# hidasib/GRU4Rec

Hardware: AMD Instinct MI355X
Metric: mini-batches/sec (gru4rec.py:661), RSC15-shaped batch=128 n_sample=2048 BPR-max (higher is better)
Workload: dtype f32

## Files before the change

gru4rec_amd/csrc/g4r_host_create.hpp:

```cpp

int g4r_device_count(void) {
    int n = 0;
    if (hipGetDeviceCount(&n) != hipSuccess) return 0;
    return n;
}
const char* g4r_last_error(void) { return g_err.c_str(); }
#ifndef G4R_HIPCC_VERSION
#define G4R_HIPCC_VERSION "unknown"
#endif
const char* g4r_version(void) { return "gru4rec_hip 0.4 (gfx950; hipcc " G4R_HIPCC_VERSION "; isa-audited)"; }
int g4r_sizeof_config(void) { return (int)sizeof(g4r_config); }

static int build_lean_args(g4r_model* m) {
    DevModel& d = m->dm;
    const StepKernels& k = m->kern;
    const int L = d.n_layers;
    std::vector<LeanV> av(L); std::vector<LeanH> ah(L); std::vector<LeanDa> aa(L); std::vector<LeanDy> ay(L);
    const bool constrained = d.embed_mode == G4R_EMBED_CONSTRAINED;
    bool any_layer = false;
    for (int l = 0; l < L; ++l) {
        if (k.fwd[l] != FWD_LEAN) continue;
        any_layer = true;
        LeanV& v = av[l]; memset(&v, 0, sizeof(v));
        v.Wx = d.dense_p + d.offWx[l]; v.Wrz = d.dense_p + d.offWrz[l]; v.Bh = d.dense_p + d.offBh[l];
// ... 42 lines not shown
        m->h_leanB = q;
        if (dalloc(m, &m->d_leanB, (size_t)1)) return -1;
        HIPCHK(hipMemcpyAsync(m->d_leanB, &m->h_leanB, sizeof(LeanB), hipMemcpyHostToDevice, m->stream));
    }
    if (k.update == UP_LEAN) {
        LeanU u; memset(&u, 0, sizeof(u));
        u.mp = nullptr; u.st = d.st; u.Wy = d.Wy; u.E = d.E; u.accWy = d.accWy; u.accE = d.accE; u.velWy = d.velWy; u.velE = d.velE;
        u.By = d.By; u.accBy = d.accBy; u.velBy = d.velBy; u.dAx = d.dAx; u.dAy = d.dAy; u.dABy = d.dABy;
        u.dense_p = d.dense_p; u.dense_acc = d.dense_acc; u.dense_vel = d.dense_vel; u.yin0 = d.yin0; u.meta = d.cur_in + 2 * d.B;
        u.dbg = d.dbgclk; u.dbgtile = d.dbgtile; u.n_items = d.n_items; u.constrained = constrained ? 1 : 0; u.wE = d.Ein; u.wY = d.Dtop;
        u.lr = d.lr; u.mom = d.mom; u.lmbd = d.lmbd;
        m->h_leanU = u;
        const std::vector<DenseTile> tiles = dense_tiles(d, 16, 64);
        m->ntiles16 = (int)tiles.size();
        const size_t nslot = cdiv((long long)G4R_OWN_SLOTS * d.R * 16 * sizeof(int), (long long)sizeof(DenseTile));
        if (dalloc(m, &m->d_tiles16, tiles.size() + nslot) || dalloc(m, &m->d_leanU, (size_t)1)) return -1;
        d.own_pos = m->sw.owner_scan_in_update ? nullptr : (int*)(m->d_tiles16 + tiles.size());
        m->h_leanU.own_on = d.own_pos ? 1 : 0;
        const bool pays = cdiv(d.R, LOSS_NW) > G4R_OWN_WINDOW_MINWG;
        m->own_window = d.own_pos && d.R <= G4R_OWN_WINDOW_MAXR && (m->sw.owner_window > 0 || (m->sw.owner_window < 0 && pays));
        HIPCHK(hipMemcpyAsync(m->d_tiles16, tiles.data(), tiles.size() * sizeof(DenseTile), hipMemcpyHostToDevice, m->stream));
        HIPCHK(hipStreamSynchronize(m->stream));
    }
    HIPCHK(hipStreamSynchronize(m->stream));
    return 0;
}

static KernelSwitches read_switches(const g4r_config& cfg) {
    KernelSwitches w;
    w.no_lean = getenv("G4R_NO_LEAN") != nullptr; w.no_mt = getenv("G4R_NO_MT") != nullptr; w.no_bmt = getenv("G4R_NO_BMT") != nullptr;
    w.no_merge = getenv("G4R_NO_MERGE") != nullptr; w.owner_scan_in_update = env_int("G4R_OWNER_SCAN", 0) != 0;
    w.owner_window = env_int("G4R_OWNER_WINDOW", -1);
    w.score_b_split = env_int("G4R_SCORE_B_SPLIT", 1) != 0;
    w.allow_lean_update = env_int("G4R_LEAN_UPDATE", 1) != 0; w.defer = env_int("G4R_DEFER", cfg.defer_updates) != 0;
    w.p2_geo = env_int("G4R_P2_GEO", -1); w.ba_geo = env_int("G4R_BA_GEO", -1);
    w.wide2 = env_int("G4R_WIDE2", -1); w.p1_ks = env_int("G4R_P1_KS", 128); w.bb_ks = env_int("G4R_BB_KS", 0);
    const char* skip = getenv("G4R_SKIP_KN");
    w.skip_kn = skip ? strtoull(skip, nullptr, 0) : 0ull;
    w.trace = getenv("G4R_TRACE") != nullptr;
    return w;
}

int g4r_create(const g4r_config* cfg, g4r_model** out) {
    if (!cfg || !out) return fail("null argument");
    if (cfg->n_layers < 1 || cfg->n_layers > G4R_MAX_LAYERS) return fail("n_layers out of range");
    if (cfg->batch_size < 1 || cfg->n_items < 1) return fail("batch_size / n_items must be positive");
    for (int l = 0; l < cfg->n_layers; ++l)
        if (cfg->layers[l] % 4 != 0 || cfg->layers[l] < 4 || cfg->layers[l] > 1024)
            return fail("layer sizes must be multiples of 4 in [4, 1024]");
    if (cfg->embed_mode == G4R_EMBED_SEPARATE && (cfg->embedding % 4 != 0 || cfg->embedding < 4 || cfg->embedding > 1024))
        return fail("embedding must be a multiple of 4 in [4, 1024]");
    if (cfg->embed_mode != G4R_EMBED_CONSTRAINED && cfg->embed_mode != G4R_EMBED_SEPARATE && cfg->embed_mode != G4R_EMBED_ONEHOT)
        return fail("unsupported embedding mode");
    if (cfg->embed_mode == G4R_EMBED_ONEHOT && 3 * cfg->layers[0] > 1024)
        return fail("one-hot input: 3 * layers[0] must be <= 1024 (row width of the Wx[0] table)");
    if (cfg->loss < 0 || cfg->loss > G4R_LOSS_XE_LOGIT) return fail("unsupported loss");
    if (cfg->smoothing != 0.f && cfg->loss != G4R_LOSS_XE && cfg->loss != G4R_LOSS_XE_LOGIT) return fail("smoothing needs a cross-entropy loss");
    if (cfg->hidden_act == G4R_ACT_SOFTMAX_LOGIT) return fail("softmax_logit is not a hidden activation");
    if (cfg->adapt < 0 || cfg->adapt > G4R_ADAPT_NONE) return fail("unknown adapt");
    if (cfg->grad_cap < 0.f) return fail("grad_cap must be >= 0");
    if (cfg->hidden_act == G4R_ACT_SOFTMAX) return fail("softmax is not a hidden activation");
    int ndev = g4r_device_count();
    if (ndev <= 0) return fail("no HIP device visible: the gfx950 path has no CPU fallback");
    if (cfg->device < 0 || cfg->device >= ndev) return fail("device ordinal out of range");
    HIPCHK(hipSetDevice(cfg->device));
    int n_cu = 0;
// ... 213 lines not shown
```

gru4rec_amd/csrc/g4r_host_debug.hpp:

```cpp
int g4r_get_debug(g4r_model* m, const char* name, float* host, int64_t count) {
    if (!m || !name || !host) return fail("null argument");
    HIPCHK(hipSetDevice(m->cfg.device));
    DevModel& d = m->dm;
    const StepKernels& k = m->kern;
    std::string s(name);
    const float* p = nullptr; int64_t n = 0;
    int l = 0;
    if (!s.empty() && isdigit((unsigned char)s.back())) { l = s.back() - '0'; s.pop_back(); }
    if (l >= d.n_layers) return fail("layer out of range");
    const int64_t bd = (int64_t)d.B * d.D[l];
    if (s == "scores") { p = d.Sc; n = (int64_t)d.B * d.ldSc; }
    else if (s == "dSx") { p = d.dSx + (size_t)((m->gstep - 1) & d.defer_mask) * (size_t)d.dSx_stride; n = (int64_t)d.B * d.Ein; }
    else if (s == "dSy") { p = d.dSy + (size_t)((m->gstep - 1) & d.defer_mask) * (size_t)d.dSy_stride; n = (int64_t)d.ldSc * d.Dtop; }
    else if (s == "dSBy") { p = d.dSBy + (size_t)((m->gstep - 1) & d.defer_mask) * (size_t)d.dSBy_stride; n = d.ldSc; }
    else if (s == "defer_stats") {
        if (count < 4) return fail("count");
        double rows = 0, bias = 0;
        if (m->defer_on) {
            std::vector<unsigned> st(2048);
            HIPCHK(hipStreamSynchronize(m->stream));
            HIPCHK(hipMemcpy(st.data(), d.dstat, st.size() * sizeof(unsigned), hipMemcpyDeviceToHost));
            for (size_t i = 0; i < st.size(); i += 2) { rows += st[i]; bias += st[i + 1]; }
        }
        host[0] = (float)rows; host[1] = (float)bias; host[2] = m->defer_on ? 1.f : 0.f; host[3] = (float)(d.defer_mask + 1);
// ... 46 lines not shown
    else if (s == "ldSc") { if (count < 1) return fail("count"); host[0] = (float)d.ldSc; return 0; }
    else if (s == "wide_mask") {
        if (count < 1) return fail("count");
        int mk = k.wide_dense ? 16 : 0;
        for (int l = 0; l < d.n_layers; ++l) mk |= k.wg[l].use;
        host[0] = (float)mk; return 0;
    }
    else if (s == "deep_geo") {
        if (count < 1) return fail("count");
        host[0] = (float)(k.p2_deep[0] + 2 * k.ba_deep[0]); return 0;
    }
    else if (s == "score_mt") { if (count < 1) return fail("count"); host[0] = k.score_fwd == SF_MT ? 272.f : 0.f; return 0; }
    else if (s == "score_bmt") { if (count < 1) return fail("count"); host[0] = (float)k.bmt_slabs; return 0; }
    else if (s == "lean") {
        if (count < 4) return fail("count");
        int mk = 0;
        for (int l = 0; l < d.n_layers; ++l) mk |= k.fwd[l] == FWD_LEAN ? 1 << l : 0;
        host[0] = (float)mk; host[1] = k.score_fwd == SF_LEAN ? 1.f : 0.f; host[2] = k.score_bwd == SB_LEAN ? 1.f : 0.f;
        host[3] = k.update == UP_LEAN ? 1.f : 0.f;
        return 0;
    }
    else if (s == "kernels") {
        const int ML = G4R_MAX_LAYERS;
        const int tail[] = {k.score_fwd, k.loss_spec, k.loss_long, k.loss_quads, k.score_bwd, k.kch, k.ksplit, k.bmt_slabs, k.update, k.chunks, k.wide_dense, k.finish_rows};
        if (count < 4 * ML + 12) return fail("count");
        for (int i = 0; i < 4 * ML + 12; ++i) host[i] = i < 4 * ML ? 0.f : (float)tail[i - 4 * ML];
        for (int l = 0; l < d.n_layers; ++l) {
            host[l] = (float)k.fwd[l]; host[ML + l] = (float)k.bwd[l]; host[2 * ML + l] = (float)(k.p2_deep[l] + 2 * k.ba_deep[l]); host[3 * ML + l] = (float)k.wg[l].use;
        }
        return 0;
    }
    else if (s == "generic") { if (count < 1) return fail("count"); host[0] = (float)d.generic; return 0; }
    else if (s == "score_b_split") { if (count < 1) return fail("count"); host[0] = (float)k.score_a_host; return 0; }
    else if (s == "n_cu") { if (count < 1) return fail("count"); host[0] = (float)m->n_cu; return 0; }
    else if (s == "ksplit") { if (count < 1) return fail("count"); host[0] = (float)d.ksplit; return 0; }
    else if (s == "dev_syncs") { if (count < 1) return fail("count"); host[0] = (float)m->n_dev_syncs; return 0; }
    else if (s == "dense_count") { if (count < 1) return fail("count"); host[0] = (float)d.dense_count; return 0; }
    else if (s == "occ_score_tile") {
        if (count < 1) return fail("count");
        int nb = 0;
        for (size_t lds = SMEM_SF2; lds >= SMEM_SF2 - 2048; lds -= 512) {
            HIPCHK(hipOccupancyMaxActiveBlocksPerMultiprocessor(&nb, (const void*)k_score_fwd_t2, GT_NTH, lds));
            fprintf(stderr, "[g4r] k_score_fwd_t2 dynamic LDS %zu -> %d workgroups per CU\n", lds, nb);
        }
        host[0] = (float)nb;
        return 0;
    }
    else if (s == "graph_mode") {
        if (count < 1) return fail("count");
        host[0] = m->gexec ? 1.f : (m->gexec_head ? 2.f : 0.f);
        return 0;
    }
    else return fail(std::string("unknown debug buffer ") + name);
    if (count != n) return fail(std::string("size mismatch for debug buffer ") + name + " expected " + std::to_string(n));
    HIPCHK(hipStreamSynchronize(m->stream));
    HIPCHK(hipMemcpy(host, p, n * sizeof(float), hipMemcpyDeviceToHost));
    return 0;
}

int g4r_debug_loss_rows(g4r_model* m, float* scores, int64_t count, int32_t M, float* lossrow) {
    if (!m || !scores || !lossrow) return fail("null argument");
    DevModel& d = m->dm;
    if (count != (int64_t)d.B * d.ldSc) return fail("size mismatch for the score rows: expected " + std::to_string((int64_t)d.B * d.ldSc));
    if (M < 1 || M > d.B) return fail("M outside [1, batch_size]");
    HIPCHK(hipSetDevice(m->cfg.device));
    HIPCHK(hipStreamSynchronize(m->stream));
// ... 158 lines not shown
```

gru4rec_amd/csrc/g4r_host_model.hpp:

```cpp
static thread_local std::string g_err;
static int fail(const std::string& s) { g_err = s; return -1; }
void g4r_set_error(const char* fmt, ...) {
    char buf[1024];
    va_list ap;
    va_start(ap, fmt);
    vsnprintf(buf, sizeof(buf), fmt, ap);
    va_end(ap);
    g_err = buf;
}
#define HIPCHK(x)                                                                                        \
    do {                                                                                                 \
        hipError_t e_ = (x);                                                                             \
        if (e_ != hipSuccess)                                                                            \
            return fail(std::string(#x) + ": " + hipGetErrorString(e_) + " @" + std::to_string(__LINE__)); \
    } while (0)
#define NCCLCHK(x)                                                                                         \
    do {                                                                                                   \
        ncclResult_t e_ = (x);                                                                             \
        if (e_ != ncclSuccess)                                                                             \
            return fail(std::string(#x) + ": " + ncclGetErrorString(e_) + " @" + std::to_string(__LINE__)); \
    } while (0)

enum { KN_GRU_P1 = 0, KN_GRU_P2, KN_SCORE_FWD, KN_LOSS, KN_SCORE_BWD, KN_BWD_PRE, KN_BWD_A, KN_BWD_B, KN_DENSE, KN_ALLREDUCE,
       KN_DENSE_APPLY, KN_SPARSE, KN_UPDATE, KN_BWD_FUSED, KN_FWD_FUSED, KN_GATE, KN_FLUSH, KN_SCAN, KN_FINISH, KN_GRU_V, KN_GRU_H, KN_GRU_DA, KN_GRU_DY, KN_OWNER_WINDOW, KN_COUNT };
static const char* KN_NAMES[KN_COUNT] = {"k_gru_p1", "k_gru_p2", "k_score_fwd", "k_loss_rows", "k_score_bwd", "k_gru_bwd_pre",
                                         "k_gru_bwd_a", "k_gru_bwd_b", "k_dense_grad", "rccl_allreduce", "k_dense_apply",
                                         "k_sparse_update", "k_update", "k_gru_bwd", "k_gru_fwd", "k_gru_gate", "k_sparse_flush", "k_defer_scan", "k_finish_rows", "k_gru_v", "k_gru_h", "k_gru_da", "k_gru_dy", "k_owner_window"};

struct EvRec { int kn; hipEvent_t a, b; };

struct KernelSwitches {
    bool no_lean = false;
    bool no_mt = false, no_bmt = false;
    bool no_merge = false;
    bool allow_lean_update = true;
    bool score_b_split = true;
    bool owner_scan_in_update = false;
    int owner_window = -1;
    bool defer = false;
    int p2_geo = -1, ba_geo = -1;
    int wide2 = -1, p1_ks = 128, bb_ks = 0;
    unsigned long long skip_kn = 0;
    bool trace = false;
};
enum GruFwdKind { FWD_LEAN = 0 , FWD_FUSED = 1 , FWD_P1S = 2 ,
                  FWD_P1_N64 = 3, FWD_P1_N32 = 4 };
enum GruBwdKind { BWD_LEAN = 0 , BWD_FUSED = 1 , BWD_ONEHOT = 2, BWD_BW = 3, BWD_B = 4 };
enum ScoreFwdKind { SF_LEAN = 0 , SF_MT = 1 , SF_T3 = 2, SF_T2 = 3, SF_K64 = 4, SF_K128 = 5  };
enum ScoreBwdKind { SB_LEAN = 0 , SB_BMT = 1 , SB_BWD2 = 2 , SB_W = 3, SB_N = 4  };
enum UpdateKind { UP_LEAN = 0 , UP_MERGED = 1 , UP_SPLIT = 2 };
struct WideGeo { int use = 0, ny = 1, nh = 1, kys = 0, khs = 0, bbn = 1, bbk = 0; };
struct StepKernels {
    int fwd[G4R_MAX_LAYERS], bwd[G4R_MAX_LAYERS];
    int p2_deep[G4R_MAX_LAYERS], ba_deep[G4R_MAX_LAYERS];
    WideGeo wg[G4R_MAX_LAYERS];
    int score_fwd;
    int loss_spec, loss_long, loss_quads;
    int score_bwd;
    int score_a_host;
    int kch, ksplit;
    int bmt_slabs;
    int nblkA, nblkB, ndtA, ndtB, nrtB;
    int update;
    int chunks;
    int wide_dense;
    int finish_rows;
};

template <class T>
struct DevBuf {
    T* p = nullptr;
    int64_t cap = 0;
    int reserve(g4r_model* m, int64_t n);
};

struct g4r_model {
    g4r_config cfg;
    DevModel dm;
    DevModel* d_dm = nullptr;
    int n_cu = 256;
    KernelSwitches sw;
    StepKernels kern;
    hipStream_t stream = nullptr;
    std::vector<void*> allocs;
    int *d_in = nullptr, *d_out = nullptr, *d_M = nullptr, *d_cmaps = nullptr;
    unsigned char* d_reset = nullptr;
    float* d_loss = nullptr;
    int64_t T = 0, loss_cap = 0;
    std::vector<int64_t> compact_steps;
    int* d_ST = nullptr;
    float *d_P = nullptr, *d_lqt = nullptr, *d_lqs = nullptr;
    int64_t gl = 0;
// ... 309 lines not shown
    }
    const bool lean_s = !sw.no_lean && Dt <= LN_MAXD && Dt % 4 == 0 && !wide && !dma && B < 65536 && d.ldSc < 65536;
    k.score_fwd = lean_s ? SF_LEAN : mt ? SF_MT : dma ? SF_T3 : (wide && Dt % T2_BK == 0) ? SF_T2 : wide ? SF_K64 : SF_K128;
    k.loss_spec = (d.final_act == G4R_ACT_ELU && d.loss == G4R_LOSS_BPR_MAX) ? 1 : (d.final_act == G4R_ACT_SOFTMAX && d.loss == G4R_LOSS_XE) ? 2
                : (d.final_act == G4R_ACT_ELU && d.loss == G4R_LOSS_TOP1_MAX) ? 3 : 0;
    k.loss_long = (size_t)(2 * d.ldSc + 18 * LOSS_NW) * sizeof(float) > (size_t)(156 * 1024);
    k.loss_quads = d.ldSc >= 4 * LOSS_T;
    const bool bwd2 = wide && Dt % 64 == 0;
    const bool top_tiles = k.bwd[top] != BWD_LEAN && k.bwd[top] != BWD_FUSED;
    if (!sw.no_bmt && bwd2 && top_tiles && Dt % 128 == 0 && Dt <= 512 && d.ldSc % BMT_WA == 0 && d.ldSc <= 0xFFFF && B <= 0xFFFF) {
        const int ntA = d.ldSc / BMT_WA * (Dt / 32), den = cdiv(B, 64) * (Dt / 128), ks = ntA / den;
        if (ntA % den == 0 && ntA % 8 == 0 && ntA <= n_cu && ntA * 8 >= n_cu * 7 && BMT_WA % (Dt / 32) == 0 && 4 * (BMT_WA / (Dt / 32)) <= 256 &&
            ks >= 2 && ks <= 24 && d.ldSc % ks == 0 && (d.ldSc / ks) % 32 == 0 && d.ldSc / ks <= 2048)
            k.bmt_slabs = ks;
    }
    k.score_bwd = (lean_s && B <= 128) ? SB_LEAN : k.bmt_slabs ? SB_BMT : bwd2 ? SB_BWD2 : wide ? SB_W : SB_N;
    k.score_a_host = (sw.score_b_split && k.score_bwd == SB_LEAN && k.bwd[top] == BWD_LEAN) ? 1 : 0;
    const int slabs_target = top_tiles ? 17 : 9;
    k.kch = GT_BK * std::max(1, (cdiv(d.ldSc, GT_BK) + slabs_target / 2) / slabs_target);
    if (k.score_bwd == SB_LEAN) k.kch = 128;
    else if (k.score_bwd == SB_BMT) k.kch = d.ldSc / k.bmt_slabs;
    else if (k.score_bwd == SB_BWD2) {
        const int ndt = Dt / 64, nrt = cdiv(B, 64), nA = cdiv(d.ldSc, 64) * ndt;
        double best = 2.0;
        for (int ks = 12; ks <= 24; ++ks) {
            const int kch = (cdiv(d.ldSc, ks) + 7) & ~7;
            if (cdiv(d.ldSc, kch) != ks) continue;
            const double rounds = (double)(nA + ks * nrt * ndt) / n_cu;
            const double waste = (std::ceil(rounds) - rounds) / std::ceil(rounds) + 1e-3 * std::abs(ks - 17);
            if (waste < best) { best = waste; k.kch = kch; }
        }
    }
    k.ksplit = cdiv(d.ldSc, k.kch);
    const int TB = wide ? 64 : 32;
    k.ndtA = cdiv(Dt + 1, TB); k.nblkA = cdiv(d.ldSc, TB) * k.ndtA;
    k.ndtB = cdiv(Dt, TB); k.nrtB = cdiv(B, TB); k.nblkB = k.ksplit * k.nrtB * k.ndtB;
    const int w = std::max(Dt, d.Ein);
    k.chunks = w <= 256 ? 1 : (w <= 512 ? 2 : 4);
    const bool dy0_parts = (k.wg[0].use & 8) != 0;
    const bool merged = !d.generic && !sw.no_merge && k.chunks <= 2 && !k.wide_dense;
    const bool lean_u = !sw.no_lean && sw.allow_lean_update && merged && d.apply_dense_inplace && B <= 128 && k.chunks == 1 && !defer_on && d.xmode == 0 &&
                        !d.touched && !dy0_parts && d.R < 65536 && cdiv(d.R, 8) < 65536 && dense_tiles(d, 16, 64).size() < 65536;
    k.update = lean_u ? UP_LEAN : merged ? UP_MERGED : UP_SPLIT;
    k.finish_rows = dy0_parts && !k.wide_dense;
    return k;
}
static int sync_dm(g4r_model* m) {
    HIPCHK(hipMemcpyAsync(m->d_dm, &m->dm, sizeof(DevModel), hipMemcpyHostToDevice, m->stream));
    HIPCHK(hipStreamSynchronize(m->stream));
    return 0;
}
```

gru4rec_amd/csrc/g4r_host_step.hpp:

```cpp
extern "C++" {
struct StepLauncher {
    g4r_model* m;
    hipStream_t s;
    std::vector<EvRec>* recs;
    size_t evi = 0;
    int kn = -1;
    hipEvent_t ev_a = nullptr, ev_b = nullptr;
    StepLauncher(g4r_model* m_, std::vector<EvRec>* recs_) : m(m_), s(m_->stream), recs(recs_) {}
    void use(int kn_, hipEvent_t a, hipEvent_t b) { kn = kn_; ev_a = a; ev_b = b; }
    void open(int kn_) {
        if (m->sw.trace) { fprintf(stderr, "[g4r] launch %s\n", KN_NAMES[kn_]); fflush(stderr); }
        use(kn_, nullptr, nullptr);
        if (!recs) return;
        while (m->evs.size() < evi + 2) { hipEvent_t e; (void)hipEventCreate(&e); m->evs.push_back(e); }
        use(kn_, m->evs[evi], m->evs[evi + 1]);
        evi += 2;
        recs->push_back(EvRec{kn_, ev_a, ev_b});
    }
    bool skipped() const { return m->sw.skip_kn && kn >= 0 && ((m->sw.skip_kn >> kn) & 1ull); }
    template <class... P, class... A>
    void launch(void (*kern)(P...), dim3 grid, dim3 block, size_t smem, A... a) {
        if (skipped()) return;
        if (ev_a) hipExtLaunchKernelGGL(kern, grid, block, (unsigned)smem, s, ev_a, ev_b, 0, static_cast<P>(a)...);
        else hipLaunchKernelGGL(kern, grid, block, smem, s, static_cast<P>(a)...);
// ... 103 lines not shown
        const bool hosted = score_a_hosted(m, lk);
        lk.launch(hosted ? k_score_b<false> : k_score_b<true>, dim3((hosted ? 0 : q.nA) + d.ksplit * q.nrb * q.ndb), dim3(512), 0, m->d_leanB, meta, d.cur_col, d.Sc,
                  d.hd[L - 1], d.Wy, d.accWy, (unsigned)d.Dtop | ((unsigned)B << 16), dimsN);
        break;
    }
    case SB_BMT:
        lk.launch(k_score_bmt, dim3(2 * (d.ldSc / BMT_WA * (d.Dtop / 32))), dim3(256), SMEM_BMT, d.Sc, d.hd[L - 1], d.Wy, d.col_item, meta, d.zrow, dmp,
                  (unsigned)d.Dtop | ((unsigned)(d.Dtop / 32) << 16), dimsN, (unsigned)B | ((unsigned)d.kch << 16), (unsigned)cdiv(B, 64) | ((unsigned)(d.Dtop / 128) << 16));
        break;
    case SB_BWD2: {
        const int ndt = d.Dtop / 64, nrt = cdiv(B, 64);
        const int nA = cdiv(d.ldSc, 64) * ndt, nB = d.ksplit * nrt * ndt, nC = cdiv(d.ldSc, 64);
        lk.launch(k_score_bwd2, dim3(nA + nB + nC), dim3(GT_NTH), (size_t)(4 * 64 * 16) * sizeof(float) + (size_t)std::max(d.kch, 64) * sizeof(int), dmp, stp, nA, nB, ndt, nrt);
        break;
    }
    case SB_W: lk.launch(k_score_bwd_w, dim3(k.nblkA + k.nblkB), dim3(GT_NTH), SMEM_SBW + (size_t)d.kch * sizeof(int), dmp, stp, k.nblkA, k.ndtA, k.ndtB, k.nrtB); break;
    default: lk.launch(k_score_bwd_n, dim3(k.nblkA + k.nblkB), dim3(GT_NTH), std::max(SMEM_TN, SMEM_NN) + (size_t)d.kch * sizeof(int), dmp, stp, k.nblkA, k.ndtA, k.ndtB, k.nrtB); break;
    }
    lk.close();
}

static void gru_backward(g4r_model* m, StepLauncher& lk, int l) {
    const DevModel& d = m->dm;
    const StepKernels& k = m->kern;
    const int L = d.n_layers, B = d.B;
    const DevModel* dmp = (const DevModel*)m->d_dm;
    StepState* stp = (StepState*)d.st;
    if (k.bwd[l] == BWD_LEAN) {
        const int nrb = cdiv(B, 16), gx = cdiv(d.IN[l], 16);
        const int* meta = d.cur_in + 2 * B;
        const LeanDa& q = m->h_leanDa[l];
        const LeanDy& y = m->h_leanDy[l];
        const unsigned dims = (unsigned)d.D[l] | ((unsigned)d.IN[l] << 16);
        lk.open(KN_GRU_DA);
        lk.launch(k_gru_da, dim3(cdiv(d.D[l], 16), nrb), dim3(128), 0, m->d_leanDa + l, meta, q.dsrc, q.Wh, q.z, q.c, q.H0, q.H1, (unsigned)d.D[l] | ((unsigned)q.ks << 16), B);
        lk.close();
        lk.open(KN_GRU_DY);
        if (score_a_hosted(m, lk) && l == L - 1) {
            const LeanB& b = m->h_leanB;
            lk.launch(k_gru_dy_a, dim3(gx, nrb + cdiv(cdiv(b.nA, 2), gx)), dim3(1024), 0, m->d_leanDy + l, meta, y.occ_idx, y.dV, y.drp, y.Wx, y.r, dims, B, m->d_leanB, d.cur_col,
                      d.Sc, d.hd[L - 1], d.accWy, (unsigned)d.Dtop | ((unsigned)B << 16), (unsigned)d.N | ((unsigned)d.ldSc << 16), (unsigned)b.nA | ((unsigned)b.ndh << 16));
        } else lk.launch(k_gru_dy, dim3(gx, nrb), dim3(1024), 0, m->d_leanDy + l, meta, y.occ_idx, y.dV, y.drp, y.Wx, y.r, dims, B);
        lk.close();
        return;
    }
    if (k.bwd[l] == BWD_FUSED) {
        lk.open(KN_BWD_FUSED);
        lk.launch(k_gru_bwd_fused, dim3(cdiv(d.IN[l], 32), cdiv(B, BF_ROWS)), dim3(512), smem_bwd_fused(d.D[l]), dmp, stp, l);
        lk.close();
        return;
    }
    lk.open(KN_BWD_PRE);
    lk.launch(k_gru_bwd_pre, dim3(cdiv((long long)B * d.D[l], 256)), dim3(256), 0, dmp, stp, l);
    lk.close();
    lk.open(KN_BWD_A);
    dim3 ga(cdiv(d.D[l], GT_BN), cdiv(B, GT_BM));
    int nfin = 0;
    if (l == L - 1 && k.score_bwd == SB_BMT) { nfin = cdiv(cdiv(d.N, 16), (int)ga.x); ga.y += nfin; }
    if (k.ba_deep[l]) lk.launch(k_gru_bwd_a_w8d, ga, dim3(512), SMEM_BA_256, dmp, stp, l, nfin);
    else lk.launch(k_gru_bwd_a_w4, ga, dim3(GT_NTH), SMEM_NT, dmp, stp, l, nfin);
    lk.close();
    lk.open(KN_BWD_B);
    const WideGeo& G = k.wg[l];
    if (k.bwd[l] == BWD_ONEHOT) lk.launch(k_onehot_step, dim3(cdiv((long long)B * d.Ein, 4 * 256)), dim3(256), 0, dmp, stp);
    else if (k.bwd[l] == BWD_BW) lk.launch(k_gru_bwd_bw, dim3(cdiv(d.IN[l], 64) * cdiv(B, 64) * G.bbn), dim3(256), SMEM_T3, dmp, stp, l, G.bbn, G.bbk);
    else lk.launch(k_gru_bwd_b, dim3(cdiv(d.IN[l], GT_BN), cdiv(B, GT_BM)), dim3(GT_NTH_FEW), SMEM_BB, dmp, stp, l);
// ... 436 lines not shown
```

gru4rec_amd/csrc/g4r_lean_kernels.cuh:

```cuda
#pragma once

#define LN_MAXD 128

__device__ __forceinline__ float ldu(const GAS float* base, unsigned boff) { return *(const GAS float*)((const GAS char*)base + boff); }
__device__ __forceinline__ int ldu_i(const GAS int* base, unsigned boff) { return *(const GAS int*)((const GAS char*)base + boff); }
__device__ __forceinline__ float4 ldu4(const GAS float* base, unsigned boff) { return *(const GAS float4*)((const GAS char*)base + boff); }
__device__ __forceinline__ void stu(GAS float* base, unsigned boff, float v) { *(GAS float*)((GAS char*)base + boff) = v; }
__device__ __forceinline__ void stu4(GAS float* base, unsigned boff, float4 v) { *(GAS float4*)((GAS char*)base + boff) = v; }

#if defined(G4R_CLK_TRACE)
#define LCLK_INIT(dbgp, slot) GAS long long* clk_ = ((dbgp) && blockIdx.x == 1 && blockIdx.y == 1 && blockIdx.z == 0 && threadIdx.x == 0) ? (dbgp) + (slot) : nullptr
#define LCLK(i) do { if (clk_) clk_[i] = wall_clock64(); } while (0)
#define LCLK_USE(x) do { if (clk_ && (x) == 123.456f) clk_[15] = 0; } while (0)
#define LSPAN_BEGIN(tilep, base) GAS long long* span_ = ((tilep) && threadIdx.x == 0) ? (tilep) + 8 * (size_t)((base) + (blockIdx.z * gridDim.y + blockIdx.y) * gridDim.x + blockIdx.x) : nullptr; \
    if (span_) span_[0] = wall_clock64()
#define LSPAN_END() do { if (span_) span_[1] = wall_clock64(); } while (0)
#define LSPAN_BEGIN_AT(tilep, idx, lead) GAS long long* span_ = ((tilep) && (lead)) ? (tilep) + 8 * (size_t)(idx) : nullptr; \
    if (span_) span_[0] = wall_clock64()
#else
#define LCLK_INIT(dbgp, slot)
#define LCLK(i)
#define LCLK_USE(x)
#define LSPAN_BEGIN(tilep, base)
#define LSPAN_END()
#define LSPAN_BEGIN_AT(tilep, idx, lead)
#endif

struct LeanV {
    GP(const float) Wx; GP(const float) Wrz; GP(const float) Bh; GP(const float) H0; GP(const float) H1;
    GP(const float) ysrc;
    GP(const int) cur_in;
    GP(float) Vc; GP(float) r; GP(float) Hr; GP(float) z; GP(float) yin0;
    GP(int) occ_idx; GP(int) occ_fl;
    GP(StepState) st;
    unsigned long long seed;
    int B, D, IN, R, first, pub_fl;
    float drop_e;
    int n_items;
    GP(long long) dbg; GP(long long) dbgtile;
// ... 458 lines not shown
    for (int rg = 0; rg < 4; ++rg) sJ[(rg * 16 + wid) * 64 + lane] = acc[rg];
    __syncthreads();
    if (wid >= 4) return;
    const LeanDy a = *ap;
    LCLK_INIT(a.dbg, 48); LCLK(6);
    LSPAN_BEGIN(a.dbgtile, 1500);
#if defined(G4R_CLK_TRACE)
    if (span_) { span_[2] = span_[0]; span_[0] = tk0; }
#endif
    float v = 0.f;
#pragma unroll
    for (int w = 0; w < 16; ++w) v += sJ[(wid * 16 + w) * 64 + lane];
    if (ncol >= IN || (int)rowe >= M) return;
    const unsigned o = 4 * (rowe * IN + ncol);
    if (a.layer0) {
        if (a.drop_e > 0.f) v *= drop_mult(a.seed, sx.g, G4R_STREAM_DROP_EMBED, rowe, ncol, 1.0f - a.drop_e);
        const float an = a2 + G4R_MUT_ACC(v * v);
        GAS float* dSx = a.dSx + (size_t)(sx.g & (unsigned)a.defer_mask) * (size_t)a.dSx_stride;
        stu(dSx, o, a.generic ? v : G4R_MUT_STEP(a.lr * v * frsq(an + G4R_EPS_ADAGRAD)));
        if (!a.generic && cnt2 == 1 && itm >= 0) a.accT[(size_t)itm * IN + ncol] = an;
        else stu(a.dAx, o, an);
    } else {
        stu(a.dylo, o, v);
    }
    LCLK(7);
    LSPAN_END();
}
__global__ __launch_bounds__(1024) void k_gru_dy(const LeanDy* __restrict__ ap, const int* meta_, const int* occ_idx_, const float* dV_, const float* drp_,
                                                 const float* Wx_, const float* r_, unsigned dims, unsigned B) {
    __shared__ float sJ[4 * 16 * 64];
    gru_dy_tile(ap, meta_, occ_idx_, dV_, drp_, Wx_, r_, dims, B, sJ);
}

template <bool LOGQ>
__global__ __launch_bounds__(256) void k_score_s(const LeanS* __restrict__ ap, const int* meta_, const int* cur_col_, const float* hd_, const float* Wy_,
                                                 const float* By_, float* Sc_, unsigned dimsA, unsigned dimsB) {
    __shared__ f32x4 sJ[4 * 4 * 64];
    const unsigned tid = threadIdx.x, lane = tid & 63, li = lane & 15, lg = lane >> 4;
    const unsigned wid = __builtin_amdgcn_readfirstlane(tid >> 6);
    const unsigned D = dimsA & 0xFFFFu, B = dimsA >> 16, N = dimsB & 0xFFFFu, ldSc = dimsB >> 16, Dq = D >> 2;
    const unsigned n0 = blockIdx.x * 32, m0 = blockIdx.y * 32;
    const GAS int* cur_col = (const GAS int*)cur_col_;
    const unsigned nA = n0 + li, nB = n0 + 16 + li;
    int it0 = ldu_i(cur_col, 4 * min(nA, ldSc - 1)), it1 = ldu_i(cur_col, 4 * min(nB, ldSc - 1));
    const int4 mt = ldi4((const GAS int*)meta_);
    const unsigned Q0 = 8 * wid + lg, Q1 = Q0 + 4;
    const bool ok0 = Q0 < Dq, ok1 = Q1 < Dq;
    const unsigned Qa = ok0 ? Q0 : 0, Qb = ok1 ? Q1 : 0;
    const GAS float* hd = (const GAS float*)hd_;
    const unsigned ra = 4 * (min(m0 + li, B - 1) * D), rb = 4 * (min(m0 + 16 + li, B - 1) * D);
    float4 a00 = ldu4(hd, ra + 16 * Qa), a01 = ldu4(hd, ra + 16 * Qb), a10 = ldu4(hd, rb + 16 * Qa), a11 = ldu4(hd, rb + 16 * Qb);
    const LeanS a = *ap;
    lean_pin(a.col_item, a.occ_idx, a.occ_fl, a.R, a.pub_fl, a.logq, a.dbg);
    LCLK_INIT(a.dbg, 56); LCLK(0);
    LSPAN_BEGIN(a.dbgtile, 4096);
    if (nA >= ldSc) it0 = -1;
    if (nB >= ldSc) it1 = -1;
    const GAS float* Wy = (const GAS float*)Wy_;
    const GAS float *w0 = Wy + (size_t)max(it0, 0) * D, *w1 = Wy + (size_t)max(it1, 0) * D;
    float4 b00 = ld4(w0 + 4 * Qa), b01 = ld4(w0 + 4 * Qb), b10 = ld4(w1 + 4 * Qa), b11 = ld4(w1 + 4 * Qb);
    const int ite = (wid & 1) ? it1 : it0;
    const unsigned ne = (wid & 1) ? nB : nA;
    float bias = ((const GAS float*)By_)[max(ite, 0)];
    if (LOGQ) {
        const DevModel& m = *a.mp;
        bias -= a.logq * (ne < B ? m.lq_tgt : m.lq_smp)[max(ite, 0)];
// ... 179 lines not shown
    for (int w = 1; w < 8; ++w) v += sJ[(wid * 8 + w) * 64 + lane];
    const unsigned b = b0 + 4 * lg + (wid & 3);
    if ((int)b < M && dq < D) st4(a.dhpart + ((size_t)kc * B + b) * D + dq, make_float4(v[0], v[1], v[2], v[3]));
    LSPAN_END();
}

template <bool ROLE_A>
__global__ __launch_bounds__(512) void k_score_b(const LeanB* __restrict__ ap, const int* meta_, const int* cur_col_, const float* Sc_, const float* hd_,
                                                 const float* Wy_, float* accWy_, unsigned dimsA, unsigned dimsB) {
    __shared__ f32x4 sJ[4 * 8 * 64];
    const unsigned tid = threadIdx.x, lane = tid & 63;
    const unsigned wid = __builtin_amdgcn_readfirstlane(tid >> 6);
    const unsigned D = dimsA & 0xFFFFu, B = dimsA >> 16, N = dimsB & 0xFFFFu, ldSc = dimsB >> 16;
    const GAS int* cur_col = (const GAS int*)cur_col_;
    const GAS float *Sc = (const GAS float*)Sc_, *hd = (const GAS float*)hd_;
    const int4 mt = ldi4((const GAS int*)meta_);
    const LeanB a = *ap;
    if (ROLE_A) {
        if (blockIdx.x < (unsigned)a.nA) { score_b_role_a(a, mt, cur_col, Sc, hd, accWy_, D, B, N, ldSc, blockIdx.x, (unsigned)a.ndh, wid, lane, sJ, true, tid == 0); return; }
        score_b_role_b(a, mt, cur_col, Sc, Wy_, D, B, ldSc, blockIdx.x - (unsigned)a.nA, wid, lane, sJ);
    } else {
        score_b_role_b(a, mt, cur_col, Sc, Wy_, D, B, ldSc, blockIdx.x, wid, lane, sJ);
    }
}
template __global__ void k_score_b<true>(const LeanB*, const int*, const int*, const float*, const float*, const float*, float*, unsigned, unsigned);
template __global__ void k_score_b<false>(const LeanB*, const int*, const int*, const float*, const float*, const float*, float*, unsigned, unsigned);

__global__ __launch_bounds__(1024) void k_gru_dy_a(const LeanDy* __restrict__ ap, const int* meta_, const int* occ_idx_, const float* dV_, const float* drp_,
                                                   const float* Wx_, const float* r_, unsigned dims, unsigned B, const LeanB* __restrict__ bp,
                                                   const int* cur_col_, const float* Sc_, const float* hd_, float* accWy_, unsigned dimsA, unsigned dimsB, unsigned tilesA) {
    __shared__ f32x4 sJ[2 * 4 * 8 * 64];
    const unsigned nrb = (B + 15) >> 4;
    if (blockIdx.y < nrb) { gru_dy_tile(ap, meta_, occ_idx_, dV_, drp_, Wx_, r_, dims, B, (float*)sJ); return; }
    const unsigned tid = threadIdx.x, lane = tid & 63;
    const unsigned wid = __builtin_amdgcn_readfirstlane(tid >> 6);
    const unsigned nA = tilesA & 0xFFFFu, half = wid >> 3;
    const unsigned t0 = 2 * ((blockIdx.y - nrb) * gridDim.x + blockIdx.x), t = t0 + half;
    if (t0 >= nA) return;
    const int4 mt = ldi4((const GAS int*)meta_);
    const LeanB a = *bp;
    const bool live = t < nA;
    score_b_role_a(a, mt, (const GAS int*)cur_col_, (const GAS float*)Sc_, (const GAS float*)hd_, accWy_, dimsA & 0xFFFFu, dimsA >> 16, dimsB & 0xFFFFu,
                   dimsB >> 16, live ? t : nA - 1, tilesA >> 16, wid & 7, lane, sJ + half * (4 * 8 * 64), live, (tid & 511) == 0);
}

template <bool MOM>
__device__ __forceinline__ void lean_rows_update(const LeanU& a, const GAS int* occ_idx, GAS int* occ_fl, const GAS float* dSx, const GAS float* dSy,
                                                 const GAS float* dSBy, const GAS int* opos_t, unsigned k, unsigned R, unsigned B) {
    const unsigned lane = threadIdx.x & 63;
    const bool tableE = k < B && !a.constrained;
    const unsigned W = tableE ? (unsigned)a.wE : (unsigned)a.wY, nc4 = W >> 2;
    const unsigned c4 = min(lane, nc4 - 1);
    const bool lok = lane < nc4;
    const unsigned kc = min(k, R - 1);
    int item = ldu_i(occ_idx, 4 * kc);
    const int opos = ldu_i(opos_t, 4 * (16 * kc + min(lane, 15u)));
    const GAS float* srow = (kc < B) ? dSx + (size_t)kc * W : dSy + (size_t)(kc - B) * W;
    const float4 sk = ld4(srow + 4 * c4);
    const bool bias = k >= B;
    const float bsk = bias ? dSBy[kc - B] : 0.f;
    lean_pin(a.Wy, a.E, a.accWy, a.accE, a.By, a.accBy, a.dAx, a.dAy, a.dABy, a.n_items, a.lr, a.mom, a.lmbd);
    if (k >= R) item = -1;
    GAS float* P = tableE ? a.E : a.Wy;
    GAS float* A = tableE ? a.accE : a.accWy;
    GAS float* V = tableE ? a.velE : a.velWy;
    const unsigned ic = (unsigned)max(item, 0);
// ... 268 lines not shown
```

Baseline: 27030.

## Fold GRU dA gate-gradient stage into the dY GEMM kernel

Adds a fused kernel that computes the candidate and update gate gradients (dA, dz) per row tile in LDS and immediately feeds them into the dY/Wx product, along with the reset-gate path through Wh. This replaces the separate k_gru_da launch followed by k_gru_dy, removing one kernel launch and the global round trip of dV between them. A variant also co-schedules the score-backward role-A tiles in the same grid. Every column block recomputes the per-row gate gradients redundantly, and only block 0 writes dV.

New measurement: 27070 (median of 2 runs). Within noise of the previous version (+0.1%).

```diff
diff --git a/gru4rec_amd/csrc/g4r_host_create.hpp b/gru4rec_amd/csrc/g4r_host_create.hpp
--- a/gru4rec_amd/csrc/g4r_host_create.hpp
+++ b/gru4rec_amd/csrc/g4r_host_create.hpp
@@ -98,6 +98,7 @@
     w.no_merge = getenv("G4R_NO_MERGE") != nullptr; w.owner_scan_in_update = env_int("G4R_OWNER_SCAN", 0) != 0;
     w.owner_window = env_int("G4R_OWNER_WINDOW", -1);
     w.score_b_split = env_int("G4R_SCORE_B_SPLIT", 1) != 0;
+    w.da_fold = env_int("G4R_DA_FOLD", 1) != 0;
     w.allow_lean_update = env_int("G4R_LEAN_UPDATE", 1) != 0; w.defer = env_int("G4R_DEFER", cfg.defer_updates) != 0;
     w.p2_geo = env_int("G4R_P2_GEO", -1); w.ba_geo = env_int("G4R_BA_GEO", -1);
     w.wide2 = env_int("G4R_WIDE2", -1); w.p1_ks = env_int("G4R_P1_KS", 128); w.bb_ks = env_int("G4R_BB_KS", 0);
diff --git a/gru4rec_amd/csrc/g4r_host_debug.hpp b/gru4rec_amd/csrc/g4r_host_debug.hpp
--- a/gru4rec_amd/csrc/g4r_host_debug.hpp
+++ b/gru4rec_amd/csrc/g4r_host_debug.hpp
@@ -102,6 +102,11 @@
     }
     else if (s == "generic") { if (count < 1) return fail("count"); host[0] = (float)d.generic; return 0; }
     else if (s == "score_b_split") { if (count < 1) return fail("count"); host[0] = (float)k.score_a_host; return 0; }
+    else if (s == "da_fold") {
+        if (count < G4R_MAX_LAYERS) return fail("count");
+        for (int l = 0; l < G4R_MAX_LAYERS; ++l) host[l] = l < d.n_layers ? (float)k.da_fold[l] : 0.f;
+        return 0;
+    }
     else if (s == "n_cu") { if (count < 1) return fail("count"); host[0] = (float)m->n_cu; return 0; }
     else if (s == "ksplit") { if (count < 1) return fail("count"); host[0] = (float)d.ksplit; return 0; }
     else if (s == "dev_syncs") { if (count < 1) return fail("count"); host[0] = (float)m->n_dev_syncs; return 0; }
diff --git a/gru4rec_amd/csrc/g4r_host_model.hpp b/gru4rec_amd/csrc/g4r_host_model.hpp
--- a/gru4rec_amd/csrc/g4r_host_model.hpp
+++ b/gru4rec_amd/csrc/g4r_host_model.hpp
@@ -35,6 +35,7 @@
     bool no_merge = false;
     bool allow_lean_update = true;
     bool score_b_split = true;
+    bool da_fold = true;
     bool owner_scan_in_update = false;
     int owner_window = -1;
     bool defer = false;
@@ -58,6 +59,7 @@
     int loss_spec, loss_long, loss_quads;
     int score_bwd;
     int score_a_host;
+    int da_fold[G4R_MAX_LAYERS];
     int kch, ksplit;
     int bmt_slabs;
     int nblkA, nblkB, ndtA, ndtB, nrtB;
@@ -433,6 +435,10 @@
         }
     }
     k.ksplit = cdiv(d.ldSc, k.kch);
+    for (int l = 0; l < L; ++l) {
+        const int planes = l == top ? k.ksplit : (k.wg[l + 1].use & 8) ? k.wg[l + 1].bbn : 1;
+        k.da_fold[l] = (sw.da_fold && k.bwd[l] == BWD_LEAN && planes <= LN_SLB && B < (1 << 24)) ? 1 : 0;
+    }
     const int TB = wide ? 64 : 32;
     k.ndtA = cdiv(Dt + 1, TB); k.nblkA = cdiv(d.ldSc, TB) * k.ndtA;
     k.ndtB = cdiv(Dt, TB); k.nrtB = cdiv(B, TB); k.nblkB = k.ksplit * k.nrtB * k.ndtB;
diff --git a/gru4rec_amd/csrc/g4r_host_step.hpp b/gru4rec_amd/csrc/g4r_host_step.hpp
--- a/gru4rec_amd/csrc/g4r_host_step.hpp
+++ b/gru4rec_amd/csrc/g4r_host_step.hpp
@@ -159,6 +159,18 @@
         const LeanDa& q = m->h_leanDa[l];
         const LeanDy& y = m->h_leanDy[l];
         const unsigned dims = (unsigned)d.D[l] | ((unsigned)d.IN[l] << 16);
+        if (k.da_fold[l] && !lk.recs) {
+            const unsigned bks = (unsigned)B | ((unsigned)q.ks << 24);
+            lk.open(KN_GRU_DY);
+            if (score_a_hosted(m, lk) && l == L - 1) {
+                const LeanB& b = m->h_leanB;
+                lk.launch(k_gru_dy_fa, dim3(gx, nrb + cdiv(cdiv(b.nA, 2), gx)), dim3(1024), 0, m->d_leanDy + l, m->d_leanDa + l, meta, y.occ_idx, q.dsrc, q.Wh, q.z, q.c, q.H0, q.H1,
+                          y.Wx, y.r, dims, bks, (unsigned)b.nA | ((unsigned)b.ndh << 16), m->d_leanB, d.cur_col, d.Sc, d.hd[L - 1], d.accWy, (unsigned)d.Dtop | ((unsigned)B << 16),
+                          (unsigned)d.N | ((unsigned)d.ldSc << 16));
+            } else lk.launch(k_gru_dy_f, dim3(gx, nrb), dim3(1024), 0, m->d_leanDy + l, m->d_leanDa + l, meta, y.occ_idx, q.dsrc, q.Wh, q.z, q.c, q.H0, q.H1, y.Wx, y.r, dims, bks);
+            lk.close();
+            return;
+        }
         lk.open(KN_GRU_DA);
         lk.launch(k_gru_da, dim3(cdiv(d.D[l], 16), nrb), dim3(128), 0, m->d_leanDa + l, meta, q.dsrc, q.Wh, q.z, q.c, q.H0, q.H1, (unsigned)d.D[l] | ((unsigned)q.ks << 16), B);
         lk.close();
diff --git a/gru4rec_amd/csrc/g4r_lean_kernels.cuh b/gru4rec_amd/csrc/g4r_lean_kernels.cuh
--- a/gru4rec_amd/csrc/g4r_lean_kernels.cuh
+++ b/gru4rec_amd/csrc/g4r_lean_kernels.cuh
@@ -5,6 +5,8 @@
 __device__ __forceinline__ float ldu(const GAS float* base, unsigned boff) { return *(const GAS float*)((const GAS char*)base + boff); }
 __device__ __forceinline__ int ldu_i(const GAS int* base, unsigned boff) { return *(const GAS int*)((const GAS char*)base + boff); }
 __device__ __forceinline__ float4 ldu4(const GAS float* base, unsigned boff) { return *(const GAS float4*)((const GAS char*)base + boff); }
+__device__ __forceinline__ float2 ldu2(const GAS float* base, unsigned boff) { return *(const GAS float2*)((const GAS char*)base + boff); }
+__device__ __forceinline__ void stu2(GAS float* base, unsigned boff, float2 v) { *(GAS float2*)((GAS char*)base + boff) = v; }
 __device__ __forceinline__ void stu(GAS float* base, unsigned boff, float v) { *(GAS float*)((GAS char*)base + boff) = v; }
 __device__ __forceinline__ void stu4(GAS float* base, unsigned boff, float4 v) { *(GAS float4*)((GAS char*)base + boff) = v; }
 
@@ -529,6 +531,209 @@
     gru_dy_tile(ap, meta_, occ_idx_, dV_, drp_, Wx_, r_, dims, B, sJ);
 }
 
+#define LN_FLD 132
+#define LN_FOLD_LDS (4 * 16 * 64 + 2 * 16 * LN_FLD)
+__device__ __forceinline__ void gru_dy_fold_tile(const LeanDy* __restrict__ ap, const LeanDa* __restrict__ qp, const int* meta_, const int* occ_idx_,
+                                                 const float* dsrc_, const float* Wh_, const float* z_, const float* c_, const float* H0_, const float* H1_,
+                                                 const float* Wx_, const float* r_, const unsigned dims, const unsigned bks, float* sJ) {
+    const unsigned tid = threadIdx.x, lane = tid & 63, li = lane & 15, lg = lane >> 4;
+    const unsigned wid = __builtin_amdgcn_readfirstlane(tid >> 6);
+    const unsigned D = dims & 0xFFFFu, IN = dims >> 16, Dq = D >> 2, B = bks & 0xFFFFFFu;
+    const int ks = (int)(bks >> 24);
+    const unsigned m0 = blockIdx.y * 16, row = m0 + li, rowB = min(row, B - 1);
+    const unsigned ncol = 16 * blockIdx.x + li, nc = min(ncol, IN - 1);
+    const unsigned rowe = m0 + 4 * lg + (wid & 3);
+    const GAS float* Wx = (const GAS float*)Wx_;
+    float* sDa = sJ + 4 * 16 * 64;
+    float* sDz = sDa + 16 * LN_FLD;
+#if defined(G4R_CLK_TRACE)
+    const long long tk0 = wall_clock64();
+    GAS long long* ck = nullptr;
+#endif
+    const unsigned prow = m0 + wid, pcol = 2 * lane;
+    const bool pcolok = pcol < D;
+    const unsigned pcolc = pcolok ? pcol : 0;
+    const unsigned poff = 4 * (min(prow, B - 1) * D + pcolc), ps = 4 * B * D;
+    const int4 mt = ldi4((const GAS int*)meta_);
+    float2 v[LN_SLB];
+#pragma unroll
+    for (int q = 0; q < LN_SLB; ++q) v[q] = ldu2((const GAS float*)dsrc_, poff + (unsigned)min(q, ks - 1) * ps);
+    const float2 z2 = ldu2((const GAS float*)z_, poff), c2 = ldu2((const GAS float*)c_, poff);
+    const float2 h20 = ldu2((const GAS float*)H0_, poff), h21 = ldu2((const GAS float*)H1_, poff);
+    const unsigned NTD = (D + 15) >> 4;
+    int itm = -1;
+    float4 b0, b1 = make_float4(0.f, 0.f, 0.f, 0.f), r4 = b1, h40 = b1, h41 = b1;
+    float4 bq[LN_PL];
+    unsigned Qs = 0;
+    bool oks = false;
+    if (wid < 8) {
+        if (wid < 4) itm = ldu_i((const GAS int*)occ_idx_, 4 * min(rowe, B - 1));
+        const unsigned part = (wid >> 2) * 2;
+        const unsigned Q0 = 8 * (wid & 3) + lg, Q1 = Q0 + 4;
+        const unsigned Qa = Q0 < Dq ? Q0 : 0, Qb = Q1 < Dq ? Q1 : 0;
+        const unsigned offw = 4 * (nc * 3 * D + part * D);
+        b0 = ldu4(Wx, offw + 16 * Qa); b1 = ldu4(Wx, offw + 16 * Qb);
+#pragma unroll
+        for (int j = 0; j < LN_PL; ++j) bq[j] = b1;
+    } else {
+        const unsigned t = wid - 8, Q0 = 4 * t + lg;
+        oks = Q0 < Dq;
+        Qs = oks ? Q0 : 0;
+        const unsigned offr = 4 * (rowB * D + 4 * Qs);
+#pragma unroll
+        for (int j = 0; j < LN_PL; ++j) {
+            const unsigned col = 16 * min((unsigned)j, NTD - 1) + 4 * lg;
+            bq[j] = ldu4((const GAS float*)Wh_, 4 * (min(16 * t + li, D - 1) * D + (col < D ? col : 0)));
+        }
+        r4 = ldu4((const GAS float*)r_, offr);
+        h40 = ldu4((const GAS float*)H0_, offr); h41 = ldu4((const GAS float*)H1_, offr);
+        b0 = ldu4(Wx, 4 * (nc * 3 * D + D) + 16 * Qs);
+    }
+    const LeanDy a = *ap;
+    const LeanDa qa = *qp;
+    lean_pin(a.accT, a.occ_fl, a.n_items, a.layer0, a.dV, qa.seed, qa.hidden_act, qa.stream, qa.ha_p0, qa.ha_p1, qa.drop_h);
+#if defined(G4R_CLK_TRACE)
+    ck = (a.dbg && blockIdx.x == 1 && blockIdx.y == 1 && (tid == 0 || tid == 512)) ? a.dbg + (tid ? 40 : 32) : nullptr;
+    if (ck) { ck[0] = tk0; ck[1] = wall_clock64(); }
+#endif
+    float a2 = 0.f;
+    int cnt2 = 0;
+    if (a.layer0 && wid < 4) {
+        const unsigned ic = min((unsigned)max(itm, 0), (unsigned)a.n_items - 1);
+        a2 = a.accT[(size_t)ic * IN + nc];
+        cnt2 = a.occ_fl[4 * (size_t)ic + 2];
+    }
+    float2 dh = make_float2(0.f, 0.f);
+#pragma unroll
+    for (int q = 0; q < LN_SLB; ++q) {
+        const float w = (q < ks) ? 1.f : 0.f;
+        dh.x = fmaf(w, v[q].x, dh.x); dh.y = fmaf(w, v[q].y, dh.y);
+    }
+    const LeanState sx = lean_state(mt);
+    const int M = sx.M;
+    if ((int)m0 >= M) return;
+    {
+        const float2 h2 = (sx.g & 1u) ? h21 : h20;
+        if (qa.drop_h > 0.f) {
+            const float4 mk = drop_mult4(qa.seed, sx.g, (unsigned)qa.stream, prow, pcolc >> 2, 1.0f - qa.drop_h);
+            const bool hi = (pcolc & 2u) != 0;
+            dh.x *= hi ? mk.z : mk.x; dh.y *= hi ? mk.w : mk.y;
+        }
+        const bool ok = (int)prow < M && pcolok;
+        const float hh[2] = {h2.x, h2.y}, zz[2] = {z2.x, z2.y}, cc[2] = {c2.x, c2.y}, dd[2] = {dh.x, dh.y};
+        float da[2], dzp[2], ad[2];
+        if (qa.hidden_act == G4R_ACT_TANH) {
+#pragma unroll
+            for (int u = 0; u < 2; ++u) ad[u] = 1.0f - cc[u] * cc[u];
+        } else {
+#pragma unroll
+            for (int u = 0; u < 2; ++u) ad[u] = act_bwd_from_out(qa.hidden_act, qa.ha_p0, qa.ha_p1, cc[u]);
+        }
+#pragma unroll
+        for (int u = 0; u < 2; ++u) {
+            const float dz = dd[u] * (cc[u] - hh[u]), dc = dd[u] * zz[u];
+            da[u] = ok ? dc * ad[u] : 0.f;
+            dzp[u] = ok ? dz * zz[u] * (1.f - zz[u]) : 0.f;
+        }
+        *(float2*)(sDa + wid * LN_FLD + pcol) = make_float2(da[0], da[1]);
+        *(float2*)(sDz + wid * LN_FLD + pcol) = make_float2(dzp[0], dzp[1]);
+        if (blockIdx.x == 0 && ok) {
+            const unsigned ov = 4 * (prow * 3 * D + pcol);
+            stu2(a.dV, ov, make_float2(da[0], da[1]));
+            stu2(a.dV, ov + 8 * D, make_float2(dzp[0], dzp[1]));
+        }
+    }
+    __syncthreads();
+#if defined(G4R_CLK_TRACE)
+    if (ck && tid == 0) { ck[2] = wall_clock64(); ck[3] = ck[2]; }
+#endif
+    f32x4 acc;
+    if (wid < 8) {
+        const float* sX = (wid >> 2) ? sDz : sDa;
+        const unsigned Q0 = 8 * (wid & 3) + lg;
+        const float4 a0 = *(const float4*)(sX + li * LN_FLD + 4 * Q0), a1 = *(const float4*)(sX + li * LN_FLD + 4 * Q0 + 16);
+        f32x4 acc0 = (f32x4){0.f, 0.f, 0.f, 0.f}, acc1 = (f32x4){0.f, 0.f, 0.f, 0.f};
+        acc0 = mfma16(a0.x, b0.x, acc0);
+        acc1 = mfma16(a0.y, b0.y, acc1);
+        acc0 = mfma16(a0.z, b0.z, acc0);
+        acc1 = mfma16(a0.w, b0.w, acc1);
+        acc0 = mfma16(a1.x, b1.x, acc0);
+        acc1 = mfma16(a1.y, b1.y, acc1);
+        acc0 = mfma16(a1.z, b1.z, acc0);
+        acc1 = mfma16(a1.w, b1.w, acc1);
+        acc = acc0 + acc1;
+#if defined(G4R_CLK_TRACE)
+        if (ck) { if (acc[0] == 123.4f) ck[15] = 0; ck[4] = wall_clock64(); }
+#endif
+    } else {
+        float4 s = make_float4(0.f, 0.f, 0.f, 0.f);
+        if (16 * (wid - 8) < D) {
+#pragma unroll
+            for (int j = 0; j < LN_PL; ++j) {
+                if ((unsigned)j < NTD) {
+                    const float4 f = *(const float4*)(sDa + li * LN_FLD + 16 * j + 4 * lg);
+                    f32x4 p = (f32x4){0.f, 0.f, 0.f, 0.f};
+                    p = mfma16(bq[j].x, f.x, p);
+                    p = mfma16(bq[j].y, f.y, p);
+                    p = mfma16(bq[j].z, f.z, p);
+                    p = mfma16(bq[j].w, f.w, p);
+                    s.x = fmaf(1.f, p[0], s.x); s.y = fmaf(1.f, p[1], s.y); s.z = fmaf(1.f, p[2], s.z); s.w = fmaf(1.f, p[3], s.w);
+                }
+            }
+        }
+#if defined(G4R_CLK_TRACE)
+        if (ck) { if (s.x == 123.4f) ck[7] = 0; ck[2] = wall_clock64(); }
+#endif
+        const float4 h4 = (sx.g & 1u) ? h41 : h40;
+        s.x *= h4.x * r4.x * (1.f - r4.x); s.y *= h4.y * r4.y * (1.f - r4.y);
+        s.z *= h4.z * r4.z * (1.f - r4.z); s.w *= h4.w * r4.w * (1.f - r4.w);
+        const bool rowok = (int)row < M;
+        if (blockIdx.x == 0 && oks && rowok) stu4(a.dV, 4 * (row * 3 * D + D + 4 * Qs), s);
+        if (!(oks && rowok)) s = make_float4(0.f, 0.f, 0.f, 0.f);
+        f32x4 acc0 = (f32x4){0.f, 0.f, 0.f, 0.f}, acc1 = (f32x4){0.f, 0.f, 0.f, 0.f};
+        acc0 = mfma16(s.x, b0.x, acc0);
+        acc1 = mfma16(s.y, b0.y, acc1);
+        acc0 = mfma16(s.z, b0.z, acc0);
+        acc1 = mfma16(s.w, b0.w, acc1);
+        acc = acc0 + acc1;
+#if defined(G4R_CLK_TRACE)
+        if (ck) { if (acc[0] == 123.4f) ck[7] = 0; ck[3] = wall_clock64(); }
+#endif
+    }
+#pragma unroll
+    for (int rg = 0; rg < 4; ++rg) sJ[(rg * 16 + wid) * 64 + lane] = acc[rg];
+    __syncthreads();
+    if (wid >= 4) return;
+    LCLK_INIT(a.dbg, 48); LCLK(6);
+    LSPAN_BEGIN(a.dbgtile, 1500);
+#if defined(G4R_CLK_TRACE)
+    if (span_) { span_[2] = span_[0]; span_[0] = tk0; }
+#endif
+    float vv = 0.f;
+#pragma unroll
+    for (int w = 0; w < 16; ++w) vv += sJ[(wid * 16 + w) * 64 + lane];
+    if (ncol >= IN || (int)rowe >= M) return;
+    const unsigned o = 4 * (rowe * IN + ncol);
+    if (a.layer0) {
+        if (a.drop_e > 0.f) vv *= drop_mult(a.seed, sx.g, G4R_STREAM_DROP_EMBED, rowe, ncol, 1.0f - a.drop_e);
+        const float an = a2 + G4R_MUT_ACC(vv * vv);
+        GAS float* dSx = a.dSx + (size_t)(sx.g & (unsigned)a.defer_mask) * (size_t)a.dSx_stride;
+        stu(dSx, o, a.generic ? vv : G4R_MUT_STEP(a.lr * vv * frsq(an + G4R_EPS_ADAGRAD)));
+        if (!a.generic && cnt2 == 1 && itm >= 0) a.accT[(size_t)itm * IN + ncol] = an;
+        else stu(a.dAx, o, an);
+    } else {
+        stu(a.dylo, o, vv);
+    }
+    LCLK(7);
+    LSPAN_END();
+}
+#define G4R_LEAN_DYF_ARGS const LeanDy* __restrict__ ap, const LeanDa* __restrict__ qp, const int* meta_, const int* occ_idx_, const float* dsrc_, \
+    const float* Wh_, const float* z_, const float* c_, const float* H0_, const float* H1_, const float* Wx_, const float* r_, unsigned dims, unsigned bks
+__global__ __launch_bounds__(1024) void k_gru_dy_f(G4R_LEAN_DYF_ARGS) {
+    __shared__ __attribute__((aligned(16))) float sJ[LN_FOLD_LDS];
+    gru_dy_fold_tile(ap, qp, meta_, occ_idx_, dsrc_, Wh_, z_, c_, H0_, H1_, Wx_, r_, dims, bks, sJ);
+}
+
 template <bool LOGQ>
 __global__ __launch_bounds__(256) void k_score_s(const LeanS* __restrict__ ap, const int* meta_, const int* cur_col_, const float* hd_, const float* Wy_,
                                                  const float* By_, float* Sc_, unsigned dimsA, unsigned dimsB) {
@@ -774,6 +979,23 @@
     __shared__ f32x4 sJ[2 * 4 * 8 * 64];
     const unsigned nrb = (B + 15) >> 4;
     if (blockIdx.y < nrb) { gru_dy_tile(ap, meta_, occ_idx_, dV_, drp_, Wx_, r_, dims, B, (float*)sJ); return; }
+    const unsigned tid = threadIdx.x, lane = tid & 63;
+    const unsigned wid = __builtin_amdgcn_readfirstlane(tid >> 6);
+    const unsigned nA = tilesA & 0xFFFFu, half = wid >> 3;
+    const unsigned t0 = 2 * ((blockIdx.y - nrb) * gridDim.x + blockIdx.x), t = t0 + half;
+    if (t0 >= nA) return;
+    const int4 mt = ldi4((const GAS int*)meta_);
+    const LeanB a = *bp;
+    const bool live = t < nA;
+    score_b_role_a(a, mt, (const GAS int*)cur_col_, (const GAS float*)Sc_, (const GAS float*)hd_, accWy_, dimsA & 0xFFFFu, dimsA >> 16, dimsB & 0xFFFFu,
+                   dimsB >> 16, live ? t : nA - 1, tilesA >> 16, wid & 7, lane, sJ + half * (4 * 8 * 64), live, (tid & 511) == 0);
+}
+__global__ __launch_bounds__(1024) void k_gru_dy_fa(G4R_LEAN_DYF_ARGS, unsigned tilesA, const LeanB* __restrict__ bp, const int* cur_col_, const float* Sc_,
+                                                    const float* hd_, float* accWy_, unsigned dimsA, unsigned dimsB) {
+    __shared__ f32x4 sJ[2 * 4 * 8 * 64];
+    static_assert(sizeof(float) * LN_FOLD_LDS <= sizeof(f32x4) * 2 * 4 * 8 * 64, "the folded tile's LDS inside role A's");
+    const unsigned nrb = ((bks & 0xFFFFFFu) + 15) >> 4;
+    if (blockIdx.y < nrb) { gru_dy_fold_tile(ap, qp, meta_, occ_idx_, dsrc_, Wh_, z_, c_, H0_, H1_, Wx_, r_, dims, bks, (float*)sJ); return; }
     const unsigned tid = threadIdx.x, lane = tid & 63;
     const unsigned wid = __builtin_amdgcn_readfirstlane(tid >> 6);
     const unsigned nA = tilesA & 0xFFFFu, half = wid >> 3;
```
